# ATTron/astroz

Measured on AMD Instinct MI355X. Metric: propagations/sec, 13,478 sats x 1,440 times, at 1/2/4/8 MI355X, higher is better.
Workload: dtype f64

## Files before the change

astroz_amd/_native.py:

```python
import ctypes as C
import os

import numpy as np

_HERE = os.path.dirname(os.path.abspath(__file__))
LIB_PATH = os.environ.get("ASTROZ_AMD_LIB") or os.path.join(_HERE, "libastroz_hip.so")

WGS84, WGS72 = 0, 1
OUT_TEME, OUT_ECEF, OUT_GEODETIC, OUT_TOPOCENTRIC = 0, 1, 2, 3
SAT_MAJOR, TIME_MAJOR = 0, 1
OUTPUT_MODES = {"teme": OUT_TEME, "ecef": OUT_ECEF, "geodetic": OUT_GEODETIC, "topocentric": OUT_TOPOCENTRIC}
PASS_DTYPE = np.dtype([("t_rise_min", "<f8"), ("t_culm_min", "<f8"), ("t_set_min", "<f8"), ("max_elevation_rad", "<f8"),
                       ("rise_azimuth_rad", "<f8"), ("set_azimuth_rad", "<f8"), ("flags", "<u4"), ("grid_rise", "<u4"),
                       ("grid_culm", "<u4"), ("grid_set", "<u4")])
PASS_UP_AT_START, PASS_UP_AT_END, PASS_CUT_BY_ERROR = 1, 2, 4
ECLIPSE_DTYPE = np.dtype([("t_entry_min", "<f8"), ("t_exit_min", "<f8"), ("flags", "<u4"), ("grid_entry", "<u4"),
                          ("grid_exit", "<u4"), ("reserved", "<u4")])
ECLIPSE_IN_AT_START, ECLIPSE_IN_AT_END, ECLIPSE_CUT_BY_ERROR = 1, 2, 4
SHADOW_UMBRA, SHADOW_PENUMBRA = 0, 1
SHADOW_KINDS = {"umbra": SHADOW_UMBRA, "penumbra": SHADOW_PENUMBRA}
ACCESS_DTYPE = np.dtype([("t_start_min", "<f8"), ("t_end_min", "<f8"), ("min_range_km", "<f8"), ("flags", "<u4"),
                         ("grid_start", "<u4"), ("grid_end", "<u4"), ("grid_min_range", "<u4")])
ACCESS_OPEN_AT_START, ACCESS_OPEN_AT_END, ACCESS_CUT_BY_ERROR = 1, 2, 4
CONJUNCTION_DTYPE = np.dtype([("t_tca_min", "<f8"), ("miss_km", "<f8"), ("rel_speed_km_s", "<f8"), ("target", "<u4"),
                              ("sat", "<u4"), ("grid_index", "<u4"), ("reserved", "<u4")])

COVERAGE_DTYPE = np.dtype([("mean_in_view", "<f8"), ("max_gap_min", "<f8"), ("n_covered", "<u4"), ("min_in_view", "<u4"),
                           ("max_in_view", "<u4"), ("n_gaps", "<u4"), ("grid_gap_start", "<u4"), ("grid_gap_end", "<u4"),
                           ("flags", "<u4"), ("reserved", "<u4")])
COVERAGE_GAP_AT_START, COVERAGE_GAP_AT_END = 1, 2

AZ_ERR_HIP = -200
PATH_ROWS_FAST, PATH_TILES_FAST, PATH_ROWS_GENERIC, PATH_LANE_SAT, PATH_DEEP_ROWS, PATH_QUASI_UNIFORM, PATH_COLS_FAST, PATH_HOST_STEP = 1, 2, 4, 8, 16, 32, 64, 128

EXPORTS = [
    "astroz_version", "astroz_init", "astroz_deinit", "tle_parse", "tle_free",
    "tle_get_satellite_number", "tle_get_epoch", "tle_get_inclination", "tle_get_eccentricity",
    "tle_get_mean_motion", "sgp4_init", "sgp4_free", "sgp4_propagate", "sgp4_propagate_batch",
    "azh_device_count", "azh_last_error", "azh_parse_tle_lines", "azh_constellation_from_tle_text",
    "azh_constellation_from_tle_lines", "azh_constellation_from_elements", "azh_constellation_subset", "azh_constellation_free",
    "azh_num_satellites", "azh_num_sgp4", "azh_num_sdp4", "azh_get_epochs", "azh_get_status",
    "azh_get_field", "azh_propagate_host", "azh_propagate_device", "azh_propagate_device_cached", "azh_propagate_device_window",
    "azh_propagate_jd_host", "azh_synchronize", "azh_propagate_one_host", "azh_set_time_tile", "azh_set_timing", "azh_set_fast_path", "azh_set_tile_kernel", "azh_set_graphs", "azh_set_f32_arithmetic", "azh_set_f32_mode",
    "azh_last_kernel_ms", "azh_last_path", "azh_last_one_stats", "azh_last_window_tiers", "azh_set_host_copy_threads", "azh_set_host_points", "azh_get_host_points", "azh_selftest_coords", "azh_selftest_host_step", "azh_host_alloc", "azh_host_free", "azh_host_pool_stats", "azh_host_pool_trim", "azh_propagate_device_f32", "azh_propagate_device_cached_f32",
    "azh_screen_target_host", "azh_screen_target_device", "azh_coarse_screen_device", "azh_coarse_screen_host",
    "azh_screen_all_host", "azh_constellation_from_omm_json", "azh_propagate_one_device", "azh_selftest_math",
    "azh_parse_tle_text", "azh_parse_omm_json", "azh_set_parse_threads", "coords_julian_to_gmst",
    "azh_group_create_from_tle_text", "azh_group_create_from_omm_json", "azh_group_free", "azh_group_num_satellites",
    "azh_group_num_devices", "azh_group_padded_rows", "azh_group_get_epochs", "azh_group_propagate_host",
    "azh_group_propagate_allgather", "azh_group_screen_target_host", "azh_group_screen_target_device", "azh_group_shard_size",
    "azh_group_shard_rows", "azh_group_synchronize", "azh_screen_track_device", "coords_eci_to_ecef", "coords_ecef_to_geodetic",
    "orbital_hohmann", "orbital_velocity", "orbital_period", "orbital_escape_velocity",
    "azh_coords_topocentric", "azh_set_observer", "azh_find_passes_host", "azh_find_passes_device",
    "azh_find_passes_stations_host", "azh_find_passes_stations_device",
    "azh_coverage_host", "azh_coverage_device",
    "azh_sun_position_teme", "azh_selftest_sun", "azh_shadow_state", "azh_find_eclipses_host", "azh_find_eclipses_device",
    "azh_line_of_sight", "azh_find_access_host", "azh_find_access_device", "azh_find_access_track_device",
    "azh_closest_approach", "azh_find_conjunctions_host", "azh_find_conjunctions_device",
]


def _stations(stations, min_elevation_deg):
    st = np.ascontiguousarray(stations, dtype=np.float64).reshape(-1, 3)
    mk = np.ascontiguousarray(np.broadcast_to(np.asarray(min_elevation_deg, dtype=np.float64), (len(st),)))
    return st, mk


# ... 163 lines not shown
    L.azh_set_f32_mode.restype = i32
    L.azh_last_kernel_ms.argtypes = [vp]
    L.azh_last_kernel_ms.restype = dbl
    L.azh_set_host_copy_threads.argtypes = [i32]
    L.azh_set_host_copy_threads.restype = None
    L.azh_set_host_points.argtypes = [sz]
    L.azh_set_host_points.restype = None
    L.azh_get_host_points.argtypes = []
    L.azh_get_host_points.restype = sz
    L.azh_host_alloc.argtypes = [C.c_size_t, C.POINTER(C.c_void_p)]
    L.azh_host_alloc.restype = i32
    L.azh_host_free.argtypes = [C.c_void_p]
    L.azh_host_free.restype = None
    L.azh_host_pool_stats.argtypes = [C.POINTER(C.c_size_t), C.POINTER(C.c_size_t)]
    L.azh_host_pool_stats.restype = None
    L.azh_host_pool_trim.argtypes = []
    L.azh_host_pool_trim.restype = None
    L.azh_last_path.argtypes = [vp]
    L.azh_last_path.restype = u32
    L.azh_last_one_stats.argtypes = [vp, vp, vp]
    L.azh_last_one_stats.restype = C.c_int32
    L.azh_last_window_tiers.argtypes = [vp, vp]
    L.azh_last_window_tiers.restype = C.c_int32
    L.azh_propagate_device_f32.argtypes = L.azh_propagate_device.argtypes
    L.azh_propagate_device_f32.restype = i32
    L.azh_propagate_device_cached_f32.argtypes = L.azh_propagate_device_cached.argtypes
    L.azh_propagate_device_cached_f32.restype = i32
    L.azh_screen_target_host.argtypes = [vp, vp, sz, vp, sz, dbl, dbl, vp, vp]
    L.azh_screen_target_host.restype = i32
    L.azh_screen_target_device.argtypes = [vp, vp, sz, vp, sz, dbl, dbl, vp, vp, vp]
    L.azh_screen_target_device.restype = i32
    L.azh_screen_track_device.argtypes = [vp, vp, sz, vp, vp, sz, dbl, vp, vp, vp]
    L.azh_screen_track_device.restype = i32
    L.azh_coarse_screen_device.argtypes = [vp, sz, sz, i32, sz, dbl, vp, vp, vp, sz, C.POINTER(sz), vp]
    L.azh_coarse_screen_device.restype = i32
    L.azh_coarse_screen_host.argtypes = [vp, sz, sz, i32, sz, dbl, vp, vp, vp, sz, C.POINTER(sz), i32]
    L.azh_coarse_screen_host.restype = i32
    L.azh_screen_all_host.argtypes = [vp, vp, sz, vp, dbl, vp, vp, sz, C.POINTER(sz)]
    L.azh_screen_all_host.restype = i32
    L.azh_coords_topocentric.argtypes = [vp, vp, dbl, vp, vp, vp]
    L.azh_coords_topocentric.restype = None
    L.azh_set_observer.argtypes = [vp, dbl, dbl, dbl]
    L.azh_set_observer.restype = i32
    L.azh_find_passes_host.argtypes = [vp, vp, sz, vp, dbl, dbl, vp, sz, vp]
    L.azh_find_passes_host.restype = i32
    L.azh_find_passes_device.argtypes = [vp, vp, sz, vp, dbl, dbl, vp, sz, vp, vp]
# ... 401 lines not shown
    def set_timing(self, enabled):
        check(lib().azh_set_timing(self._h, 1 if enabled else 0), "azh_set_timing")

    def synchronize(self):
        check(lib().azh_synchronize(self._h), "azh_synchronize")

    def last_kernel_ms(self):
        return lib().azh_last_kernel_ms(self._h)

    def last_path(self):
        return int(lib().azh_last_path(self._h))

    def last_one_stats(self):
        a, b = C.c_uint32(0), C.c_uint32(0)
        check(lib().azh_last_one_stats(self._h, C.byref(a), C.byref(b)), "azh_last_one_stats")
        return int(a.value), int(b.value)


    def last_window_tiers(self):
        cnt = (C.c_uint32 * 4)()
        check(lib().azh_last_window_tiers(self._h, cnt), "azh_last_window_tiers")
        return dict(zip(("general", "eps", "ecc", "rejected"), (int(x) for x in cnt)))


class DeviceGroup:

    def __init__(self, text, devices, grav=WGS72, n_chunks=4):
        b = text.encode() if isinstance(text, str) else bytes(text)
        dv = (C.c_int32 * len(devices))(*devices)
        h = C.c_void_p()
        fn = lib().azh_group_create_from_omm_json if b.lstrip()[:1] in (b"{", b"[") else lib().azh_group_create_from_tle_text
        check(fn(b, len(b), grav, dv, len(devices), n_chunks, C.byref(h)), "azh_group_create")
        self._h = h
        self.n = lib().azh_group_num_satellites(h)
        self.n_devices = lib().azh_group_num_devices(h)
        self.padded_rows = lib().azh_group_padded_rows(h)
        self.epochs = np.empty(self.n)
        check(lib().azh_group_get_epochs(h, self.epochs.ctypes.data), "azh_group_get_epochs")

    def close(self):
        if getattr(self, "_h", None):
            lib().azh_group_free(self._h)
            self._h = None

    def __del__(self):
        try:
# ... 281 lines not shown
```

astroz_amd/csrc/astroz_hip.hip:

```cpp
#include "../../include/astroz_hip.h"

#include <hip/hip_runtime.h>
#include <dlfcn.h>
#include <rccl/rccl.h>

#include <algorithm>
#include <atomic>
#include <cmath>
#include <condition_variable>
#include <deque>
#include <map>
#include <cstdio>
#include <cstdlib>
#include <cstring>
#include <mutex>
#include <new>
#include <memory>
#include <string>
#include <thread>
#include <type_traits>
#include <vector>

#include "kernels.h"
#include "passes_kernel.h"
// ... 109 lines not shown
        own_ = true;
        return Create(&h_, flags);
    }
    void borrow(H h)
    {
        reset();
        h_ = h;
        own_ = false;
    }
    void reset()
    {
        if (h_ && own_) (void)Destroy(h_);
        h_ = nullptr;
    }
    bool owned() const { return h_ && own_; }
    operator H() const { return h_; }

  private:
    H h_ = nullptr;
    bool own_ = false;
};
using Stream = HipHandle<hipStream_t, hipStreamCreateWithFlags, hipStreamDestroy>;
using Event = HipHandle<hipEvent_t, hipEventCreateWithFlags, hipEventDestroy>;

constexpr int kStageSlots = 3;
constexpr size_t kStageChunk = size_t(16) << 20;
struct HostStager {
    Event ev[kStageSlots];
    PinnedBuf slot[kStageSlots];
    int32_t ensure()
    {
        for (int k = 0; k < kStageSlots; ++k) {
            if (slot[k].ensure(kStageChunk) != AZ_OK) return AZ_ERR_HIP;
            if (!ev[k] && !hip_ok(ev[k].create(hipEventDisableTiming), "hipEventCreate")) return AZ_ERR_HIP;
        }
        return AZ_OK;
    }
};
}

struct azh_constellation {
    int device = 0;
    size_t n = 0, n_pad = 0;
    AzGrav g{};
    Stream s_main, s_deep, s_ecc;
    Event ev_fork, ev_join, ev_fork2, ev_join2, ev_t0, ev_t1;
    Event ev_one;
    Event ev_graph;
    DevBuf<double> d_el;
    DevBuf<unsigned> d_flags;
    std::vector<unsigned> h_flags;
    std::vector<double> h_epoch;
    std::vector<double> h_raw[AZ_NUM_RAW];
    DevBuf<unsigned> d_list;
    std::vector<unsigned> h_list;
    unsigned n_sgp4 = 0, n_sdp4 = 0, n_bad = 0;
    DevBuf<double> d_times, d_offsets, d_sin, d_cos, d_seeds;
    DevBuf<double> d_node_cache;
    struct FastPlan {
        bool valid = false, mixed32 = false;
        unsigned tile_c = 0, tile_e = 0, n_list = 0, n_seg = 0, parity = 0;
        DevBuf<double> win;
        DevBuf<unsigned char> flag;
        DevBuf<unsigned> redo;
    } plan[4];
    int last_plan = -1;
    DevBuf<double> d_inc;
    DevBuf<double> d_fast_rec;
    double uniform_step = 0.0;
    DevBuf<float> d_delta;
    double delta_max = 0.0;
    std::vector<float> h_delta;
    DevBuf<double> d_delta64;
    std::vector<double> h_delta64;
    bool delta_wide = false;
    double grid_t0 = 0.0;
    unsigned last_path = 0;
    DevBuf<double> d_tgt, d_part_d2, d_out_d;
    DevBuf<unsigned> d_part_t, d_out_t;
    DevBuf<double> d_one_t, d_one_o;
    DevBuf<unsigned char> d_one_e;
    DevBuf<unsigned> d_one_items;
    unsigned one_segments = 0;
    PinnedBuf h_stage;
    std::vector<double> h_times, h_offsets;
    std::vector<uint8_t> h_mask;
    double staged_ref_jd = 0.0;
    hipStream_t staged_stream = nullptr;
// ... 90 lines not shown
    hipStream_t s = nullptr;
    if (!hip_ok(hipStreamCreateWithFlags(&s, hipStreamNonBlocking), "hipStreamCreate")) return nullptr;
    streams[device] = s;
    return s;
}

void drop_graphs(azh_constellation *c);

int32_t build(const std::vector<double> (&cols)[AZ_NUM_RAW], size_t n, int grav, int device, azh_constellation **out)
{
    if (!out) return AZ_ERR_NULL_POINTER;
    *out = nullptr;
    if (n == 0) return AZ_ERR_VALUE;
    if (n > 0x7fffffffu) return AZ_ERR_VALUE;
    int ndev = 0;
    HIP_TRY(hipGetDeviceCount(&ndev));
    if (device < 0 || device >= ndev) {
        g_last_error = "no such HIP device";
        return AZ_ERR_HIP;
    }
    std::unique_ptr<azh_constellation> c(new (std::nothrow) azh_constellation());
    if (!c) return AZ_ERR_ALLOC_FAILED;
    c->device = device;
    c->n = n;
    c->n_pad = (n + 63) / 64 * 64;
    c->g = make_grav(grav);
    if (set_device(c.get()) != AZ_OK) return AZ_ERR_HIP;
    if (n > 16) {
        if (!hip_ok(c->s_main.create(hipStreamNonBlocking), "hipStreamCreate") ||
            !hip_ok(c->s_deep.create(hipStreamNonBlocking), "hipStreamCreate") ||
            !hip_ok(c->s_ecc.create(hipStreamNonBlocking), "hipStreamCreate") ||
            !hip_ok(c->ev_graph.create(hipEventDisableTiming | hipEventDisableSystemFence), "hipEventCreate"))
            return AZ_ERR_HIP;
    } else {
        c->s_main.borrow(small_stream(device));
        if (!c->s_main) return AZ_ERR_HIP;
        c->s_deep.borrow(c->s_main);
        c->s_ecc.borrow(c->s_main);
    }
    for (Event *e : {&c->ev_fork2, &c->ev_join2, &c->ev_fork, &c->ev_join, &c->ev_one})
        if (!hip_ok(e->create(hipEventDisableTiming), "hipEventCreate")) return AZ_ERR_HIP;
    if (!hip_ok(c->ev_t0.create(hipEventDefault), "hipEventCreate") || !hip_ok(c->ev_t1.create(hipEventDefault), "hipEventCreate"))
        return AZ_ERR_HIP;
    const size_t np = c->n_pad;
    DevBuf<double> d_raw;
    if (c->d_el.ensure((size_t)AZ_NUM_FIELDS * np) != AZ_OK || c->d_flags.ensure(np) != AZ_OK || d_raw.ensure((size_t)AZ_NUM_RAW * np) != AZ_OK)
// ... 231 lines not shown
    if (a.mode != AZ_OUT_TEME) tile = std::min(tile, (unsigned)AZ_TILE_SEG_MAX);
    if (a.delta || a.delta64) tile = std::min(tile, (unsigned)AZ_DELTA_SEG);
    f.tile_c = f.tile_e = tile;
    f.kind = 2;
    return f;
}

template <bool VEL, int FRAME, int SINK, bool ECC>
void launch_rows_fast(const PropArgs &a, unsigned n_slots, hipStream_t st)
{
    with_delta(a.delta_wide ? 2 : (a.delta ? 1 : 0), [&](auto DELTA) {
        hipLaunchKernelGGL((k_rows_fast<VEL, FRAME, SINK, ECC, DELTA>), dim3(pad8(n_slots), cgrid_y(a.n_times, a.tile)), dim3(64), 0, st, a);
    });
}
PropArgs ecc_part(const PropArgs &a, unsigned tile)
{
    PropArgs e = a;
    e.list = a.list + a.n_circ;
    e.n_list = a.n_list - a.n_circ;
    e.tile = tile;
    e.redo_slot0 = a.n_circ;
    return e;
}
template <bool VEL, int FRAME, int SINK>
void launch_redo(const PropArgs &a, dim3 grid, hipStream_t st)
{
    hipLaunchKernelGGL((k_rows<VEL, gen_frame(FRAME), SINK, true>), grid, dim3(64), 0, st, a);
}

int32_t launch_near_fast(const PropArgs &a, bool vel, const FastShape &shape, dim3 rgrid, hipStream_t st, const EccSide &side)
{
    PropArgs e = ecc_part(a, shape.tile_e), c = a;
    c.n_list = a.n_circ;
    c.tile = shape.tile_c;
    unsigned n_e = e.n_list, n_c = c.n_list;
    if (a.row_lo > 0 || a.row_hi < a.n_rows) {
        c.slot_lo = a.win_circ_lo; c.slot_hi = a.win_circ_hi; n_c = c.slot_hi - c.slot_lo;
        e.slot_lo = a.win_ecc_lo; e.slot_hi = a.win_ecc_hi; n_e = e.slot_hi - e.slot_lo;
        if (c.slot_hi == 0) c.n_list = n_c = 0;
        if (e.slot_hi == 0) e.n_list = n_e = 0;
    }
    const bool beside = side.stream != nullptr && n_c;
    const hipStream_t se = beside ? side.stream : st;
    if (beside)
        if (int32_t rc = stream_after(se, st, side.fork); rc != AZ_OK) return rc;
    with_outputs(a, vel, [&](auto VEL, auto FRAME, auto SINK) {
        if (n_e) launch_rows_fast<VEL, FRAME, SINK, true>(e, n_e, se);
        launch_redo<VEL, FRAME, SINK>(a, rgrid, se);
        if (n_c && FRAME == 0 && shape.packed32)
            with_bool(shape.mixed32, [&](auto MIXED) {
                with_bool(a.delta != nullptr, [&](auto DELTA) {
                    hipLaunchKernelGGL((k_rows_fast32<VEL, MIXED, DELTA>), dim3(pad8(n_c), cgrid_y(a.n_times, c.tile)), dim3(64), 0, st, c);
                });
            });
        else if (n_c)
            launch_rows_fast<VEL, FRAME, SINK, false>(c, n_c, st);
    });
    return beside ? stream_after(st, se, side.join) : AZ_OK;
}

void launch_tiles(const PropArgs &a0, bool vel, hipStream_t st, const FastShape &shape)
{
    PropArgs a = a0, r = a0;
    a.tile = r.tile = shape.tile_c;
    r.tm_rows = 1;
    const dim3 grid(pad8((a.n_rows + 15u) / 16u), cgrid_y(a.n_times, a.tile));
    with_vel_frame(vel, a.mode, [&](auto VEL, auto FRAME) {
        with_bool(a.delta64 != nullptr, [&](auto WIDE) {
            hipLaunchKernelGGL((k_tiles_fast<VEL, FRAME, WIDE ? 2 : 0>), grid, dim3(1024), 0, st, a);
        });
        launch_redo<VEL, FRAME, AZ_SINK_F64>(r, dim3(256, 4), st);
// ... 93 lines not shown
    }
    if (c->d_times.ensure(n_times) != AZ_OK) return AZ_ERR_HIP;
    HIP_TRY(hipMemcpyAsync(c->d_times.p, times, sizeof(double) * n_times, hipMemcpyHostToDevice, st));
    c->have_offsets = offsets != nullptr;
    if (offsets) {
        if (c->d_offsets.ensure(c->n) != AZ_OK) return AZ_ERR_HIP;
        HIP_TRY(hipMemcpyAsync(c->d_offsets.p, offsets, sizeof(double) * c->n, hipMemcpyHostToDevice, st));
    }
    c->have_mask = mask != nullptr;
    if (mask) {
        if (c->d_mask.ensure(c->n) != AZ_OK) return AZ_ERR_HIP;
        HIP_TRY(hipMemcpyAsync(c->d_mask.p, mask, c->n, hipMemcpyHostToDevice, st));
    }
    if (mode != AZ_OUT_TEME) {
        if (c->d_sin.ensure(n_times) != AZ_OK || c->d_cos.ensure(n_times) != AZ_OK) return AZ_ERR_HIP;
        hipLaunchKernelGGL(k_gmst, dim3((unsigned)((n_times + 255) / 256)), dim3(256), 0, st, c->d_times.p,
                           (unsigned)n_times, reference_jd, c->d_sin.p, c->d_cos.p);
        HIP_TRY(hipGetLastError());
    }
    c->cached_n_times = (unsigned)n_times;
    c->cached_mode = mode;
    c->seeds_valid = false;
    drop_graphs(c);
    for (auto &pl : c->plan) pl.valid = false;
    c->last_plan = -1;
    c->uniform_step = 0.0;
    c->delta_max = 0.0;
    c->delta_wide = false;
    c->grid_t0 = n_times ? times[0] : 0.0;
    if (n_times >= 2) {
        double t0 = times[0], step = (times[n_times - 1] - t0) / (double)(n_times - 1);
        double tmax = std::max(std::fabs(t0), std::fabs(times[n_times - 1]));
        const double tol = 4.0 * 2.220446049250313e-16 * std::max(tmax, std::fabs(step));
        bool uni = std::isfinite(step) && step != 0.0;
        double dmax = 0.0;
        for (size_t i = 1; uni && i < n_times; ++i) {
            dmax = std::max(dmax, std::fabs(times[i] - std::fma((double)i, step, t0)));
            uni = dmax <= AZ_DELTA_MAX;
        }
        if (uni && dmax > tol) {
            c->h_delta.assign(n_times + AZ_DELTA_SEG, 0.0f);
            for (size_t i = 0; i < n_times; ++i) c->h_delta[i] = (float)(times[i] - std::fma((double)i, step, t0));
            if (c->d_delta.ensure(c->h_delta.size()) != AZ_OK) return AZ_ERR_HIP;
            HIP_TRY(hipMemcpyAsync(c->d_delta.p, c->h_delta.data(), sizeof(float) * c->h_delta.size(), hipMemcpyHostToDevice, st));
            c->h_delta64.assign(n_times + AZ_DELTA_SEG, 0.0);
            for (size_t i = 0; i < n_times; ++i) c->h_delta64[i] = times[i] - std::fma((double)i, step, t0);
            if (c->d_delta64.ensure(c->h_delta64.size()) != AZ_OK) return AZ_ERR_HIP;
// ... 90 lines not shown
    if (!pl.valid || pl.tile_c != shape.tile_c || pl.tile_e != shape.tile_e || pl.n_list != n_list || pl.mixed32 != shape.mixed32) {
        if (c->capturing) return AZ_RC_EAGER;
        drop_graphs(c);
        const size_t items = (size_t)n_list * n_seg + ((size_t)a.n_times + 63) / 64 * (c->n_sgp4 - c->n_circ);
        if (pl.redo.cap < 4 + 3 * items || pl.win.cap < (size_t)n_list * n_seg * AZ_PLAN_NUM) HIP_TRY(hipStreamSynchronize(st));
        if (pl.redo.ensure(4 + 3 * items) != AZ_OK || pl.win.ensure((size_t)n_list * n_seg * AZ_PLAN_NUM) != AZ_OK ||
            pl.flag.ensure((size_t)n_list * n_seg) != AZ_OK)
            return AZ_ERR_HIP;
        HIP_TRY(hipMemsetAsync(pl.redo.p, 0, 4 * sizeof(unsigned), st));
        HIP_TRY(hipMemsetAsync(pl.flag.p, 0, (size_t)n_list * n_seg, st));
        PlanArgs q{};
        q.el = a.el; q.flags = a.flags; q.n_pad = a.n_pad; q.list = a.list; q.n_list = n_list; q.n_circ = a.n_circ;
        q.n_times = a.n_times; q.tile_c = shape.tile_c; q.tile_e = shape.tile_e; q.by_flags = shape.kind == 2 ? 1u : 0u;
        q.times = a.times; q.offsets = a.offsets; q.inc = a.inc; q.step = a.uniform_step; q.dt_mult = shape.kind == 1 ? 128.0 : 64.0;
        q.delta_max = (a.delta || a.delta64) ? a.delta_max : 0.0;
        q.grid_t0 = a.grid_t0;
        q.f32_mixed = shape.mixed32 ? 1u : 0u;
        q.win = pl.win.p; q.flag = pl.flag.p;
        q.redo_static = pl.redo.p + 2; q.redo_c0 = pl.redo.p; q.redo_c1 = pl.redo.p + 1; q.redo_items = pl.redo.p + 4;
        q.g = a.g;
        hipLaunchKernelGGL(k_plan_windows, dim3((n_list + 255) / 256, n_seg), dim3(256), 0, st, q);
        hipLaunchKernelGGL(k_plan_arm, dim3(1), dim3(64), 0, st, q.redo_static, q.redo_c0, q.redo_c1);
        HIP_TRY(hipGetLastError());
        pl.valid = true;
        pl.tile_c = shape.tile_c; pl.tile_e = shape.tile_e; pl.n_list = n_list; pl.n_seg = n_seg; pl.parity = 0; pl.mixed32 = shape.mixed32;
    }
    c->last_plan = (int)shape.kind;
    a.plan_win = pl.win.p;
    a.plan_flag = pl.flag.p;
    a.plan_stride = n_list;
    a.redo_static = pl.redo.p + 2;
    a.redo_count = pl.redo.p + pl.parity;
    a.redo_next = pl.redo.p + (pl.parity ^ 1u);
    a.redo_items = pl.redo.p + 4;
    pl.parity ^= 1u;
    return AZ_OK;
}

void drop_graphs(azh_constellation *c)
{
    if (c->graphs.empty()) return;
    if (hipEventSynchronize(c->ev_graph) != hipSuccess) (void)hipGetLastError();
    for (auto &g : c->graphs) {
        if (g.exec) (void)hipGraphExecDestroy(g.exec);
        if (g.graph) (void)hipGraphDestroy(g.graph);
    }
// ... 5 lines not shown
{
    (void)hipSetDevice(device);
    drop_graphs(this);
}

namespace {
unsigned plan_sig(const azh_constellation *c)
{
    unsigned s = 0;
    for (unsigned k = 0; k < 4; ++k) s |= (c->plan[k].parity & 1u) << k;
    return s;
}

int32_t launch_all(azh_constellation *c, double *d_pos, double *d_vel, int layout, size_t stride, uint8_t *d_err,
                   hipStream_t st, int f32 = 0, size_t row_lo = 0, size_t row_hi = ~(size_t)0)
{
    const unsigned n_times = c->cached_n_times;
    if (n_times == 0) return AZ_OK;
    row_hi = std::min(row_hi, c->n);
    if (row_lo >= row_hi) return AZ_OK;
    if (stride == 0) stride = c->n;
    if (layout == AZ_LAYOUT_TIME_MAJOR && stride < c->n) return AZ_ERR_VALUE;
    c->last_plan = -1;

    PropArgs a{};
    a.el = c->d_el.p;
    a.flags = c->d_flags.p;
    a.n_pad = c->n_pad;
    a.times = c->d_times.p;
    a.n_times = n_times;
    a.offsets = c->have_offsets ? c->d_offsets.p : nullptr;
    a.pos = d_pos;
    a.vel = d_vel;
    a.sin_g = c->d_sin.p;
    a.cos_g = c->d_cos.p;
    a.mask = c->have_mask ? c->d_mask.p : nullptr;
    a.err = d_err;
    a.stride_sats = stride;
    a.mode = c->cached_mode;
    if (a.mode == AZ_OUT_TOPOCENTRIC) {
        if (c->obs_dirty) {
            if (c->capturing) return AZ_RC_EAGER;
            if (c->d_obs.ensure(1) != AZ_OK) return AZ_ERR_HIP;
            HIP_TRY(hipMemcpyAsync(c->d_obs.p, &c->obs, sizeof(AzObserver), hipMemcpyHostToDevice, st));
            c->obs_dirty = false;
        }
// ... 88 lines not shown
        if (tiles && fork) HIP_TRY(hipStreamWaitEvent(st, c->ev_join, 0));
        if (tiles && !cols) a.list = c->d_list.p + c->off_cat;
        FastShape shape;
        const bool fast = a.inc != nullptr && (tiles || use_rows(a, layout, false));
        if (fast) {
            if (!tiles || cols) a.list = c->d_list.p + c->off_circ;
            a.n_list = c->n_sgp4;
            a.n_circ = c->n_circ;
            a.rowmap = c->d_list.p + (cols ? c->off_rowmap2 : c->off_rowmap);
            a.n_rows = (unsigned)c->n;
            shape = cols ? fast_shape_cols(a, (unsigned)c->n, c->n_sgp4, c->n_circ)
                         : (tiles ? fast_shape_tiles(a, (unsigned)c->n) : fast_shape_rows(a, c->n_sgp4, c->n_circ));
            if (int32_t rc = ensure_plan(c, a, shape, st); rc != AZ_OK) return rc;
        }
        const EccSide side{c->s_ecc, c->ev_fork2, c->ev_join2};
        if (a.n_list > 0 && cols) {
            if (int32_t rc = launch_cols(a, d_vel != nullptr, st, shape, side, c->n_sdp4); rc != AZ_OK) return rc;
            path |= AZH_PATH_COLS_FAST;
        } else if (a.n_list > 0 && tiles) {
            launch_tiles(a, d_vel != nullptr, st, shape);
            path |= AZH_PATH_TILES_FAST;
        } else if (a.n_list > 0 && fast) {
            const dim3 rgrid(std::min(8192u, std::max(256u, (a.n_list * cgrid_y(a.n_times, shape.tile_c) + 63u) / 64u)), 4);
            if (int32_t rc = launch_near_fast(a, d_vel != nullptr, shape, rgrid, st, side); rc != AZ_OK) return rc;
            path |= AZH_PATH_ROWS_FAST;
        } else if (a.n_list > 0) {
            path |= launch_propagate(a, layout, d_vel != nullptr, false, st);
        }
        if ((a.delta || a.delta64) && (path & (AZH_PATH_TILES_FAST | AZH_PATH_ROWS_FAST | AZH_PATH_COLS_FAST))) path |= AZH_PATH_QUASI_UNIFORM;
        HIP_TRY(hipGetLastError());
    }
    if (c->n_bad > 0) {
        hipLaunchKernelGGL(k_fill_bad, dim3((n_times + 255) / 256, c->n_bad), dim3(256), 0, st,
                           c->d_list.p + c->n_sgp4 + c->n_sdp4, c->n_bad, c->d_flags.p, n_times, d_pos, d_vel, d_err,
                           c->have_mask ? c->d_mask.p : nullptr, layout, stride, f32, a.row_lo, a.row_hi);
        HIP_TRY(hipGetLastError());
    }
    if (fork && !tiles) HIP_TRY(hipStreamWaitEvent(st, c->ev_join, 0));
    c->last_path = path;
    if (c->timing) {
        HIP_TRY(hipEventRecord(c->ev_t1, st));
        c->timed = true;
    }
    return AZ_OK;
}

int32_t launch_cached(azh_constellation *c, double *d_pos, double *d_vel, int layout, size_t stride, uint8_t *d_err, hipStream_t st,
// ... 689 lines not shown
    if (!c) return AZ_ERR_NULL_POINTER;
    c->tile_kernel = enabled != 0;
    c->cols_kernel = enabled == 2 ? 1 : (enabled == 1 ? 0 : c->cols_kernel);
    drop_graphs(c);
    return AZ_OK;
}

int32_t azh_set_fast_path(azh_constellation *c, int32_t enabled)
{
    if (!c) return AZ_ERR_NULL_POINTER;
    c->fast_path = enabled != 0;
    drop_graphs(c);
    return AZ_OK;
}

int32_t azh_set_time_tile(azh_constellation *c, uint32_t sgp4_tile, uint32_t sdp4_tile)
{
    if (!c) return AZ_ERR_NULL_POINTER;
    c->tile_sgp4 = sgp4_tile;
    c->tile_sdp4 = sdp4_tile;
    drop_graphs(c);
    return AZ_OK;
}

int32_t azh_set_graphs(azh_constellation *c, int32_t enabled)
{
    if (!c) return AZ_ERR_NULL_POINTER;
    c->graphs_on = enabled != 0;
    if (!c->graphs_on) drop_graphs(c);
    return AZ_OK;
}

static int32_t propagate_device(azh_constellation *c, const double *times, size_t n_times, const double *offsets, double *d_pos,
                                double *d_vel, int32_t mode, double reference_jd, const uint8_t *mask, int32_t layout, size_t stride,
                                uint8_t *d_err, void *stream, int f32)
{
    return guarded([&]() -> int32_t {
        if (!c || !d_pos || (n_times && !times)) return AZ_ERR_NULL_POINTER;
        if (mode < 0 || mode > AZ_OUT_TOPOCENTRIC || layout < 0 || layout > 1) return AZ_ERR_VALUE;
        if (mode == AZ_OUT_TOPOCENTRIC && !c->have_observer) return AZ_ERR_VALUE;
        if (n_times == 0) return AZ_OK;
        if (set_device(c) != AZ_OK) return AZ_ERR_HIP;
        hipStream_t st = stream ? (hipStream_t)stream : c->s_main;
        int32_t rc = stage_inputs(c, times, n_times, offsets, mask, mode, reference_jd, st);
        if (rc != AZ_OK) return rc;
        return launch_all(c, d_pos, d_vel, layout, stride, d_err, st, f32);
// ... 1963 lines not shown
```

astroz_amd/csrc/kernels.h:

```cpp
#pragma once
#include <hip/hip_runtime.h>

#include <type_traits>

#include "init_device.h"
#include "propagate_device.h"
#include "fast_step.h"
#include "fast_step_f32.h"

#ifndef AZ_BLOCK
#define AZ_BLOCK 256
#endif
#ifndef AZ_PROP_FAST
#define AZ_PROP_FAST 1
#endif
#ifndef AZ_MIN_WAVES
#define AZ_MIN_WAVES 1
#endif
#ifndef AZ_ROWS_WAVES
#define AZ_ROWS_WAVES 3
#endif
#ifndef AZ_DEEP_WAVES
#define AZ_DEEP_WAVES 2
#endif
#define AZ_RESEED 256
#ifndef AZ_SM_CHUNK
#define AZ_SM_CHUNK 4
#endif

struct PropArgs {
    const double *el;
    const unsigned *flags;
    size_t n_pad;
    const unsigned *list;
    unsigned n_list;
    const double *times;
    unsigned n_times;
    const double *offsets;
    double *pos, *vel;
    const double *sin_g, *cos_g;
// ... 1230 lines not shown
                }
            } else {
                if (live_a) {
                    const az_f3s a = {r[0].x, r[1].x, r[2].x};
                    __builtin_nontemporal_store(a, reinterpret_cast<az_f3s *>(prow + (size_t)i * 3));
                    if (VEL) {
                        const az_f3s b = {v[0].x, v[1].x, v[2].x};
                        __builtin_nontemporal_store(b, reinterpret_cast<az_f3s *>(vrow + (size_t)i * 3));
                    }
                }
                if (live_b) {
                    const az_f3s a = {r[0].y, r[1].y, r[2].y};
                    __builtin_nontemporal_store(a, reinterpret_cast<az_f3s *>(prow + (size_t)(i + 1) * 3));
                    if (VEL) {
                        const az_f3s b = {v[0].y, v[1].y, v[2].y};
                        __builtin_nontemporal_store(b, reinterpret_cast<az_f3s *>(vrow + (size_t)(i + 1) * 3));
                    }
                }
            }
        }
    }
}

template <bool VEL, int FRAME, int SINK, bool REDO = false>
__global__ void __launch_bounds__(64, AZ_ROWS_WAVES) k_rows(PropArgs p)
{
    typedef typename std::conditional<SINK == AZ_SINK_F32, float, double>::type out_t;
    const unsigned lane = threadIdx.x;
    __shared__ __attribute__((aligned(16))) double rows_lds[AZ_ROWS_TLDS + C_NUM_MAX + 2 + 8];
    static_assert(F_nodeo < 8 && F_argpo < 8 && F_mo < 8, "the epoch angles sit in the first eight rows of the element table");
    constexpr bool redo = REDO;
    const unsigned n_items = redo ? *p.redo_count : 1u;
#pragma unroll 1
    for (unsigned item = redo ? blockIdx.x : 0u; item < n_items; item += redo ? gridDim.x : 1u) {
    unsigned row, t_lo, t_hi;
    if (redo) {
        row = p.redo_items[3 * (size_t)item];
        const unsigned b0 = p.redo_items[3 * (size_t)item + 1], b1 = p.redo_items[3 * (size_t)item + 2];
        const unsigned quarter = (((b1 - b0 + 63) / 64 + gridDim.y - 1) / gridDim.y) * 64;
        t_lo = b0 + blockIdx.y * quarter;
        t_hi = min(t_lo + quarter, b1);
        if (t_lo >= b1) continue;
    } else {
        row = az_list_slot(p);
        if (row >= az_list_end(p)) return;
        t_lo = blockIdx.y * p.tile;
        t_hi = min(t_lo + p.tile, p.n_times);
    }
    const unsigned s = p.list[row];
    const unsigned fl = p.flags[s];
    if (SINK != AZ_SINK_SCREEN && ((p.mask != nullptr && p.mask[s] == 0) || s < p.row_lo || s >= p.row_hi)) continue;
    const double off = az_uniform(p.offsets ? p.offsets[s] : 0.0);
    const RotK rk = az_rotk();
#if defined(AZ_ABLATE) && AZ_ABLATE == 3
// ... 574 lines not shown
```

bindings/zig/astroz_hip.zig:

```

pub const HipError = error{
    BadTleLength,
    BadChecksum,
    DeepSpaceNotSupported,
    InvalidEccentricity,
    SatelliteDecayed,
    ValueError,
    OutOfMemory,
    NullPointer,
    NotInitialized,
    DeviceFailure,
    Unknown,
};

pub fn check(rc: i32) HipError!void {
    return switch (rc) {
        0 => {},
        -1 => HipError.BadTleLength,
        -2 => HipError.BadChecksum,
        -10 => HipError.DeepSpaceNotSupported,
        -11 => HipError.InvalidEccentricity,
        -12 => HipError.SatelliteDecayed,
        -20 => HipError.ValueError,
        -100 => HipError.OutOfMemory,
// ... 68 lines not shown
pub extern "c" fn azh_parse_tle_text(text: [*]const u8, len: usize, out16: [*]f64, max_records: usize, n_found: *usize) i32;
pub extern "c" fn azh_parse_omm_json(text: [*]const u8, len: usize, out16: [*]f64, max_records: usize, n_found: *usize) i32;
pub extern "c" fn azh_set_parse_threads(n: i32) void;
pub extern "c" fn azh_constellation_from_omm_json(text: [*]const u8, len: usize, grav: i32, device: i32, out: *?*Handle) i32;
pub extern "c" fn azh_constellation_subset(h: ?*const Handle, indices: [*]const u32, n: usize, device: i32, out: *?*Handle) i32;

pub extern "c" fn azh_propagate_device_window(h: ?*Handle, row_lo: usize, row_hi: usize, d_pos: [*]f64, d_vel: ?[*]f64, layout: i32,
    out_stride_sats: usize, d_err: ?[*]u8, stream: ?*anyopaque) i32;
pub extern "c" fn azh_set_f32_mode(h: ?*Handle, mode: i32) i32;
pub extern "c" fn azh_set_f32_arithmetic(h: ?*Handle, enabled: i32) i32;
pub extern "c" fn azh_set_fast_path(h: ?*Handle, enabled: i32) i32;
pub extern "c" fn azh_set_tile_kernel(h: ?*Handle, enabled: i32) i32;
pub extern "c" fn azh_set_graphs(h: ?*Handle, enabled: i32) i32;
pub extern "c" fn azh_set_host_points(n: usize) void;
pub extern "c" fn azh_get_host_points() usize;
pub extern "c" fn azh_set_host_copy_threads(n: i32) void;
pub extern "c" fn azh_host_alloc(bytes: usize, out: *?*anyopaque) i32;
pub extern "c" fn azh_host_free(p: ?*anyopaque) void;
pub extern "c" fn azh_host_pool_stats(live_bytes: ?*usize, free_bytes: ?*usize) void;
pub extern "c" fn azh_host_pool_trim() void;
pub extern "c" fn azh_last_path(h: ?*const Handle) u32;
pub extern "c" fn azh_last_one_stats(h: ?*Handle, n_segments: ?*u32, n_handed_over: ?*u32) i32;
pub extern "c" fn azh_last_window_tiers(h: ?*Handle, counts: *[4]u32) i32;
pub extern "c" fn azh_propagate_one_device(h: ?*Handle, sat_index: usize, d_tsince_min: [*]const f64, n: usize, d_pos: [*]f64,
    d_vel: ?[*]f64, d_err: ?[*]u8, stream: ?*anyopaque) i32;
pub extern "c" fn azh_selftest_math(x: [*]const f64, n: usize, out6n: [*]f64, device: i32) i32;
pub extern "c" fn azh_selftest_host_step(el: [*]const f64, n_pad: usize, sat: usize, flags: u32, grav: i32, tsince_min: [*]const f64, n: usize,
    out6n: [*]f64, err: ?[*]u8) i32;
pub extern "c" fn azh_selftest_coords(op: i32, in: *const [4]f64, out: *[5]f64) i32;

pub extern "c" fn coords_julian_to_gmst(jd: f64) f64;
pub extern "c" fn coords_eci_to_ecef(eci: *const [3]f64, gmst: f64, ecef: *[3]f64) void;
pub extern "c" fn coords_ecef_to_geodetic(ecef: *const [3]f64, lla: *[3]f64) void;
pub extern "c" fn azh_coords_topocentric(r_teme: *const [3]f64, v_teme: ?*const [3]f64, gmst: f64, observer_lla: *const [3]f64,
    aer: *[3]f64, aer_rate: ?*[3]f64) void;

pub const OUT_TOPOCENTRIC: i32 = 3;
pub const Pass = extern struct {
    t_rise_min: f64,
    t_culm_min: f64,
    t_set_min: f64,
    max_elevation_rad: f64,
    rise_azimuth_rad: f64,
    set_azimuth_rad: f64,
    flags: u32,
    grid_rise: u32,
// ... 124 lines not shown
```

include/astroz_hip.h:

```cpp
#ifndef ASTROZ_HIP_H
#define ASTROZ_HIP_H

#include <stddef.h>
#include <stdint.h>

#ifdef __cplusplus
extern "C" {
#endif

enum {
    AZ_OK = 0,
    AZ_ERR_BAD_TLE_LENGTH = -1,
    AZ_ERR_BAD_CHECKSUM = -2,
    AZ_ERR_DEEP_SPACE_NOT_SUPPORTED = -10,
    AZ_ERR_INVALID_ECCENTRICITY = -11,
    AZ_ERR_SATELLITE_DECAYED = -12,
    AZ_ERR_VALUE = -20,
    AZ_ERR_ALLOC_FAILED = -100,
    AZ_ERR_NULL_POINTER = -101,
    AZ_ERR_NOT_INITIALIZED = -102,
    AZ_ERR_HIP = -200,
    AZ_ERR_UNKNOWN = -999
};

// ... 244 lines not shown
                                       double *const *d_min_dist_km, uint32_t *const *d_min_t_index);
size_t azh_group_shard_size(const azh_group *g, int32_t device_slot);
int32_t azh_group_shard_rows(const azh_group *g, int32_t device_slot, uint32_t *out_rows);
int32_t azh_group_synchronize(azh_group *g);

int32_t azh_propagate_jd_host(azh_constellation *c, const double *jd, const double *fr, size_t n_times,
                              double *pos, double *vel, int32_t output_mode, int32_t layout, uint8_t *err);
int32_t azh_synchronize(azh_constellation *c);

int32_t azh_propagate_one_host(azh_constellation *c, size_t sat_index, const double *tsince_min, size_t n,
                               double *pos, double *vel, uint8_t *err);

int32_t azh_propagate_one_device(azh_constellation *c, size_t sat_index, const double *d_tsince_min, size_t n,
                                 double *d_pos, double *d_vel, uint8_t *d_err, void *stream);
int32_t azh_selftest_math(const double *x, size_t n, double *out6n, int32_t device);
int32_t azh_selftest_coords(int32_t op, const double in[4], double out[5]);
int32_t azh_selftest_host_step(const double *el, size_t n_pad, size_t sat, uint32_t flags, int32_t grav, const double *tsince_min,
                               size_t n, double *out6n, uint8_t *err);

int32_t azh_set_time_tile(azh_constellation *c, uint32_t sgp4_tile, uint32_t sdp4_tile);
int32_t azh_set_fast_path(azh_constellation *c, int32_t enabled);
int32_t azh_set_tile_kernel(azh_constellation *c, int32_t enabled);
int32_t azh_set_graphs(azh_constellation *c, int32_t enabled);
void azh_set_host_copy_threads(int32_t n);
void azh_set_host_points(size_t n);
size_t azh_get_host_points(void);
int32_t azh_host_alloc(size_t bytes, void **out);
void azh_host_free(void *p);
void azh_host_pool_stats(size_t *live_bytes, size_t *free_bytes);
void azh_host_pool_trim(void);
int32_t azh_set_timing(azh_constellation *c, int32_t enabled);
double azh_last_kernel_ms(azh_constellation *c);
#define AZH_PATH_ROWS_FAST 1u
#define AZH_PATH_TILES_FAST 2u
#define AZH_PATH_ROWS_GENERIC 4u
#define AZH_PATH_LANE_SAT 8u
#define AZH_PATH_DEEP_ROWS 16u
#define AZH_PATH_COLS_FAST 64u
#define AZH_PATH_QUASI_UNIFORM 32u
#define AZH_PATH_HOST_STEP 128u
uint32_t azh_last_path(const azh_constellation *c);
int32_t azh_last_one_stats(azh_constellation *c, uint32_t *n_segments, uint32_t *n_handed_over);
#define AZH_WINDOW_TIER_GENERAL 0
#define AZH_WINDOW_TIER_EPS 1
#define AZH_WINDOW_TIER_ECC 2
#define AZH_WINDOW_TIER_REJECTED 3
// ... 8 lines not shown
```

Baseline: 96.21 billion.

## Size redo kernel grid from async plan count and add slim occupancy variant

```diff
diff --git a/astroz_amd/_native.py b/astroz_amd/_native.py
--- a/astroz_amd/_native.py
+++ b/astroz_amd/_native.py
@@ -42,7 +42,7 @@
     "azh_num_satellites", "azh_num_sgp4", "azh_num_sdp4", "azh_get_epochs", "azh_get_status",
     "azh_get_field", "azh_propagate_host", "azh_propagate_device", "azh_propagate_device_cached", "azh_propagate_device_window",
     "azh_propagate_jd_host", "azh_synchronize", "azh_propagate_one_host", "azh_set_time_tile", "azh_set_timing", "azh_set_fast_path", "azh_set_tile_kernel", "azh_set_graphs", "azh_set_f32_arithmetic", "azh_set_f32_mode",
-    "azh_last_kernel_ms", "azh_last_path", "azh_last_one_stats", "azh_last_window_tiers", "azh_set_host_copy_threads", "azh_set_host_points", "azh_get_host_points", "azh_selftest_coords", "azh_selftest_host_step", "azh_host_alloc", "azh_host_free", "azh_host_pool_stats", "azh_host_pool_trim", "azh_propagate_device_f32", "azh_propagate_device_cached_f32",
+    "azh_last_kernel_ms", "azh_last_path", "azh_last_one_stats", "azh_last_window_tiers", "azh_set_redo_grid", "azh_last_redo_grid", "azh_set_host_copy_threads", "azh_set_host_points", "azh_get_host_points", "azh_selftest_coords", "azh_selftest_host_step", "azh_host_alloc", "azh_host_free", "azh_host_pool_stats", "azh_host_pool_trim", "azh_propagate_device_f32", "azh_propagate_device_cached_f32",
     "azh_screen_target_host", "azh_screen_target_device", "azh_coarse_screen_device", "azh_coarse_screen_host",
     "azh_screen_all_host", "azh_constellation_from_omm_json", "azh_propagate_one_device", "azh_selftest_math",
     "azh_parse_tle_text", "azh_parse_omm_json", "azh_set_parse_threads", "coords_julian_to_gmst",
@@ -252,6 +252,10 @@
     L.azh_last_one_stats.restype = C.c_int32
     L.azh_last_window_tiers.argtypes = [vp, vp]
     L.azh_last_window_tiers.restype = C.c_int32
+    L.azh_set_redo_grid.argtypes = [vp, u32, u32, u32]
+    L.azh_set_redo_grid.restype = i32
+    L.azh_last_redo_grid.argtypes = [vp]
+    L.azh_last_redo_grid.restype = u32
     L.azh_propagate_device_f32.argtypes = L.azh_propagate_device.argtypes
     L.azh_propagate_device_f32.restype = i32
     L.azh_propagate_device_cached_f32.argtypes = L.azh_propagate_device_cached.argtypes
@@ -699,6 +703,12 @@
         check(lib().azh_last_window_tiers(self._h, cnt), "azh_last_window_tiers")
         return dict(zip(("general", "eps", "ecc", "rejected"), (int(x) for x in cnt)))
 
+    def set_redo_grid(self, lo=0, reserve=0, cap=0):
+        check(lib().azh_set_redo_grid(self._h, lo, reserve, cap), "azh_set_redo_grid")
+
+    def last_redo_grid(self):
+        return int(lib().azh_last_redo_grid(self._h))
+
 
 class DeviceGroup:
 
diff --git a/astroz_amd/csrc/astroz_hip.hip b/astroz_amd/csrc/astroz_hip.hip
--- a/astroz_amd/csrc/astroz_hip.hip
+++ b/astroz_amd/csrc/astroz_hip.hip
@@ -155,6 +155,35 @@
 };
 using Stream = HipHandle<hipStream_t, hipStreamCreateWithFlags, hipStreamDestroy>;
 using Event = HipHandle<hipEvent_t, hipEventCreateWithFlags, hipEventDestroy>;
+
+struct AsyncWord {
+    unsigned *h = nullptr;
+    Event ev;
+    bool pending = false;
+    AsyncWord() = default;
+    AsyncWord(const AsyncWord &) = delete;
+    AsyncWord &operator=(const AsyncWord &) = delete;
+    ~AsyncWord() { if (h) (void)hipHostFree(h); }
+    bool landed()
+    {
+        if (!pending) return true;
+        if (hipEventQuery(ev) == hipSuccess) pending = false;
+        else (void)hipGetLastError();
+        return !pending;
+    }
+    bool request(const unsigned *d_word, hipStream_t st)
+    {
+        if (!landed()) return false;
+        if (!h && hipHostMalloc((void **)&h, sizeof(unsigned), hipHostMallocDefault) != hipSuccess) { h = nullptr; (void)hipGetLastError(); return false; }
+        if (!ev && ev.create(hipEventDisableTiming) != hipSuccess) { (void)hipGetLastError(); return false; }
+        if (hipMemcpyAsync(h, d_word, sizeof(unsigned), hipMemcpyDeviceToHost, st) != hipSuccess || hipEventRecord(ev, st) != hipSuccess) {
+            (void)hipGetLastError();
+            return false;
+        }
+        pending = true;
+        return true;
+    }
+};
 
 constexpr int kStageSlots = 3;
 constexpr size_t kStageChunk = size_t(16) << 20;
@@ -196,7 +225,18 @@
         DevBuf<double> win;
         DevBuf<unsigned char> flag;
         DevBuf<unsigned> redo;
+        AsyncWord count;
+        bool count_asked = false;
+        int n_static = -1;
+        void invalidate() { valid = false; count_asked = false; n_static = -1; }
+        int static_items()
+        {
+            if (n_static < 0 && count_asked && count.landed()) n_static = (int)std::min(*count.h, 0x7fffffffu);
+            return n_static;
+        }
     } plan[4];
+    unsigned redo_lo = 0, redo_reserve = 0, redo_cap = 0;
+    unsigned last_redo_grid = 0;
     int last_plan = -1;
     DevBuf<double> d_inc;
     DevBuf<double> d_fast_rec;
@@ -333,6 +373,7 @@
     std::unique_ptr<azh_constellation> c(new (std::nothrow) azh_constellation());
     if (!c) return AZ_ERR_ALLOC_FAILED;
     c->device = device;
+    if (const char *e = getenv("ASTROZ_AMD_REDO_GRID")) (void)sscanf(e, "%u,%u,%u", &c->redo_lo, &c->redo_reserve, &c->redo_cap);
     c->n = n;
     c->n_pad = (n + 63) / 64 * 64;
     c->g = make_grav(grav);
@@ -610,14 +651,28 @@
     e.redo_slot0 = a.n_circ;
     return e;
 }
-template <bool VEL, int FRAME, int SINK>
+template <bool VEL, int FRAME, int SINK, int REDO = AZ_REDO_FULL>
 void launch_redo(const PropArgs &a, dim3 grid, hipStream_t st)
 {
-    hipLaunchKernelGGL((k_rows<VEL, gen_frame(FRAME), SINK, true>), grid, dim3(64), 0, st, a);
-}
-
-int32_t launch_near_fast(const PropArgs &a, bool vel, const FastShape &shape, dim3 rgrid, hipStream_t st, const EccSide &side)
-{
+    hipLaunchKernelGGL((k_rows<VEL, gen_frame(FRAME), SINK, REDO>), grid, dim3(64), 0, st, a);
+}
+struct RedoSize {
+    int n_static = -1;
+    unsigned lo = 0, reserve = 0, cap = 0;
+    unsigned grid = 0;
+};
+constexpr unsigned AZ_REDO_LO = 16, AZ_REDO_RESERVE = 64, AZ_REDO_CAP = 8192;
+constexpr unsigned AZ_REDO_SLIM_ITEMS = 1024;
+inline unsigned redo_blocks(unsigned items, const RedoSize &z)
+{
+    const unsigned cap = std::max(z.cap, 1u);
+    return std::min(cap, std::max(std::min(items, cap), std::max(z.lo, 1u)));
+}
+
+int32_t launch_near_fast(const PropArgs &a, bool vel, const FastShape &shape, dim3 rgrid, hipStream_t st, const EccSide &side,
+                         RedoSize *sized = nullptr)
+{
+    RedoSize none, &rz = sized ? *sized : none;
     PropArgs e = ecc_part(a, shape.tile_e), c = a;
     c.n_list = a.n_circ;
     c.tile = shape.tile_c;
@@ -634,7 +689,14 @@
         if (int32_t rc = stream_after(se, st, side.fork); rc != AZ_OK) return rc;
     with_outputs(a, vel, [&](auto VEL, auto FRAME, auto SINK) {
         if (n_e) launch_rows_fast<VEL, FRAME, SINK, true>(e, n_e, se);
-        launch_redo<VEL, FRAME, SINK>(a, rgrid, se);
+        rz.grid = rz.n_static >= 0 ? redo_blocks((unsigned)rz.n_static + rz.reserve, rz) : rgrid.x;
+        bool slim = false;
+        if constexpr (decltype(FRAME)::value == 0 && decltype(VEL)::value)
+            slim = rz.n_static >= 0 && (unsigned)rz.n_static + rz.reserve <= AZ_REDO_SLIM_ITEMS && beside && !shape.packed32 && !a.delta && !a.delta64;
+        if constexpr (decltype(FRAME)::value == 0 && decltype(VEL)::value) {
+            if (slim) launch_redo<VEL, FRAME, SINK, AZ_REDO_SLIM>(a, dim3(rz.grid, rgrid.y), se);
+        }
+        if (!slim) launch_redo<VEL, FRAME, SINK>(a, dim3(rz.grid, rgrid.y), se);
         if (n_c && FRAME == 0 && shape.packed32)
             with_bool(shape.mixed32, [&](auto MIXED) {
                 with_bool(a.delta != nullptr, [&](auto DELTA) {
@@ -774,7 +836,7 @@
     c->cached_mode = mode;
     c->seeds_valid = false;
     drop_graphs(c);
-    for (auto &pl : c->plan) pl.valid = false;
+    for (auto &pl : c->plan) pl.invalidate();
     c->last_plan = -1;
     c->uniform_step = 0.0;
     c->delta_max = 0.0;
@@ -911,6 +973,8 @@
         hipLaunchKernelGGL(k_plan_windows, dim3((n_list + 255) / 256, n_seg), dim3(256), 0, st, q);
         hipLaunchKernelGGL(k_plan_arm, dim3(1), dim3(64), 0, st, q.redo_static, q.redo_c0, q.redo_c1);
         HIP_TRY(hipGetLastError());
+        pl.invalidate();
+        pl.count_asked = pl.count.request(q.redo_static, st);
         pl.valid = true;
         pl.tile_c = shape.tile_c; pl.tile_e = shape.tile_e; pl.n_list = n_list; pl.n_seg = n_seg; pl.parity = 0; pl.mixed32 = shape.mixed32;
     }
@@ -962,6 +1026,7 @@
     if (stride == 0) stride = c->n;
     if (layout == AZ_LAYOUT_TIME_MAJOR && stride < c->n) return AZ_ERR_VALUE;
     c->last_plan = -1;
+    c->last_redo_grid = 0;
 
     PropArgs a{};
     a.el = c->d_el.p;
@@ -1096,7 +1161,13 @@
             path |= AZH_PATH_TILES_FAST;
         } else if (a.n_list > 0 && fast) {
             const dim3 rgrid(std::min(8192u, std::max(256u, (a.n_list * cgrid_y(a.n_times, shape.tile_c) + 63u) / 64u)), 4);
-            if (int32_t rc = launch_near_fast(a, d_vel != nullptr, shape, rgrid, st, side); rc != AZ_OK) return rc;
+            RedoSize rz;
+            rz.n_static = c->capturing ? -1 : c->plan[shape.kind].static_items();
+            rz.lo = c->redo_lo ? c->redo_lo : AZ_REDO_LO;
+            rz.reserve = c->redo_reserve ? c->redo_reserve : AZ_REDO_RESERVE;
+            rz.cap = c->redo_cap ? c->redo_cap : AZ_REDO_CAP;
+            if (int32_t rc = launch_near_fast(a, d_vel != nullptr, shape, rgrid, st, side, &rz); rc != AZ_OK) return rc;
+            c->last_redo_grid = rz.grid;
             path |= AZH_PATH_ROWS_FAST;
         } else if (a.n_list > 0) {
             path |= launch_propagate(a, layout, d_vel != nullptr, false, st);
@@ -1832,6 +1903,18 @@
     drop_graphs(c);
     return AZ_OK;
 }
+
+int32_t azh_set_redo_grid(azh_constellation *c, uint32_t lo, uint32_t reserve, uint32_t cap)
+{
+    if (!c) return AZ_ERR_NULL_POINTER;
+    c->redo_lo = lo;
+    c->redo_reserve = reserve;
+    c->redo_cap = cap;
+    drop_graphs(c);
+    return AZ_OK;
+}
+
+uint32_t azh_last_redo_grid(const azh_constellation *c) { return c ? c->last_redo_grid : 0u; }
 
 int32_t azh_set_graphs(azh_constellation *c, int32_t enabled)
 {
diff --git a/astroz_amd/csrc/kernels.h b/astroz_amd/csrc/kernels.h
--- a/astroz_amd/csrc/kernels.h
+++ b/astroz_amd/csrc/kernels.h
@@ -16,6 +16,11 @@
 #endif
 #ifndef AZ_MIN_WAVES
 #define AZ_MIN_WAVES 1
+#endif
+#define AZ_REDO_FULL 1
+#define AZ_REDO_SLIM 2
+#ifndef AZ_REDO_SLIM_WAVES
+#define AZ_REDO_SLIM_WAVES 5
 #endif
 #ifndef AZ_ROWS_WAVES
 #define AZ_ROWS_WAVES 3
@@ -1292,14 +1297,14 @@
     }
 }
 
-template <bool VEL, int FRAME, int SINK, bool REDO = false>
-__global__ void __launch_bounds__(64, AZ_ROWS_WAVES) k_rows(PropArgs p)
+template <bool VEL, int FRAME, int SINK, int REDO = 0>
+__global__ void __launch_bounds__(64, REDO == AZ_REDO_SLIM ? AZ_REDO_SLIM_WAVES : AZ_ROWS_WAVES) k_rows(PropArgs p)
 {
     typedef typename std::conditional<SINK == AZ_SINK_F32, float, double>::type out_t;
     const unsigned lane = threadIdx.x;
     __shared__ __attribute__((aligned(16))) double rows_lds[AZ_ROWS_TLDS + C_NUM_MAX + 2 + 8];
     static_assert(F_nodeo < 8 && F_argpo < 8 && F_mo < 8, "the epoch angles sit in the first eight rows of the element table");
-    constexpr bool redo = REDO;
+    constexpr bool redo = REDO != 0;
     const unsigned n_items = redo ? *p.redo_count : 1u;
 #pragma unroll 1
     for (unsigned item = redo ? blockIdx.x : 0u; item < n_items; item += redo ? gridDim.x : 1u) {
diff --git a/bindings/zig/astroz_hip.zig b/bindings/zig/astroz_hip.zig
--- a/bindings/zig/astroz_hip.zig
+++ b/bindings/zig/astroz_hip.zig
@@ -114,6 +114,8 @@
 pub extern "c" fn azh_last_path(h: ?*const Handle) u32;
 pub extern "c" fn azh_last_one_stats(h: ?*Handle, n_segments: ?*u32, n_handed_over: ?*u32) i32;
 pub extern "c" fn azh_last_window_tiers(h: ?*Handle, counts: *[4]u32) i32;
+pub extern "c" fn azh_set_redo_grid(h: ?*Handle, lo: u32, reserve: u32, cap: u32) i32;
+pub extern "c" fn azh_last_redo_grid(h: ?*const Handle) u32;
 pub extern "c" fn azh_propagate_one_device(h: ?*Handle, sat_index: usize, d_tsince_min: [*]const f64, n: usize, d_pos: [*]f64,
     d_vel: ?[*]f64, d_err: ?[*]u8, stream: ?*anyopaque) i32;
 pub extern "c" fn azh_selftest_math(x: [*]const f64, n: usize, out6n: [*]f64, device: i32) i32;
diff --git a/include/astroz_hip.h b/include/astroz_hip.h
--- a/include/astroz_hip.h
+++ b/include/astroz_hip.h
@@ -290,6 +290,9 @@
 int32_t azh_set_fast_path(azh_constellation *c, int32_t enabled);
 int32_t azh_set_tile_kernel(azh_constellation *c, int32_t enabled);
 int32_t azh_set_graphs(azh_constellation *c, int32_t enabled);
+
+int32_t azh_set_redo_grid(azh_constellation *c, uint32_t lo, uint32_t reserve, uint32_t cap);
+uint32_t azh_last_redo_grid(const azh_constellation *c);
 void azh_set_host_copy_threads(int32_t n);
 void azh_set_host_points(size_t n);
 size_t azh_get_host_points(void);
```

After: 97.06 billion (median of 6 runs). No clear change (+0.9%).
